# johndpope/OmniHuman-1-hack

Measured on AMD Instinct MI355X. Metric: DiT denoising steps/sec + VAE frames/sec, Wan2.1-1.3B 480x832 81f, higher is better.
Workload: dtype bf16; 1 GPU; Wan2.1-T2V-1.3B 50-step sample, 81f 480x832, latent [16, 21, 60, 104], S=32760, CFG step; weights=random-init (xavier) Wan2.1-T2V-1.3B architecture, parallelism=dp1: replicas, one clip per GPU, no data-path collective

## Files before the change

### omnihuman-1-hack_amd/csrc/dit_elementwise.hip

```cpp
#include "omh_common.h"
#include <mutex>
#include <stdio.h>
#include <string.h>
#include <stdlib.h>

namespace {

constexpr int MAXV_GENERIC = 32;

template <int MAXV, int LN_RPW>
__global__ __launch_bounds__(256)
void layernorm_modulate_kernel(const float* __restrict__ x, uint16_t* __restrict__ y, int64_t rows, int dim,
                               float eps, float mul_const, const float* __restrict__ mul0,
                               const float* __restrict__ mul1, int64_t mul1_stride,
                               const float* __restrict__ add0, const float* __restrict__ add1,
                               int64_t add1_stride, int64_t rows_per_batch) {
    const int lane = threadIdx.x & 63;
    const int64_t row0 = ((int64_t)blockIdx.x * 4 + (threadIdx.x >> 6)) * LN_RPW;
    if (row0 >= rows) return;
    const int nv = dim >> 2;
    float4 mu[MAXV], ad[MAXV], v[MAXV], nx[MAXV];
    int64_t have = -1;
#pragma unroll
    for (int i = 0; i < MAXV; ++i) {
// ... 111 lines not shown
    const float4* wv = (const float4*)weight;
    uint2* yr = (uint2*)(y + row * dim);
    const bool same_pairs = rot && (256 % head_dim) == 0;
    float cs2[2] = {1.f, 1.f}, sn2[2] = {0.f, 0.f};
    if (same_pairs) {
        const int p0 = ((4 * lane) % head_dim) >> 1;
#pragma unroll
        for (int e = 0; e < 2; ++e) {
            const int pc = p0 + e;
            const int pos = pc < cf ? pf : (pc < cf + c3 ? ph : pw);
            const int idx = min(pos, rope_len - 1) * hc + pc;
            cs2[e] = rope_cos[idx]; sn2[e] = rope_sin[idx];
        }
    }
#pragma unroll
    for (int i = 0; i < MAXV; ++i) {
        const int c = lane + 64 * i;
        if (c < nv) {
            float4 t = v[i];
            t.x *= rinv; t.y *= rinv; t.z *= rinv; t.w *= rinv;
            if (wv) { const float4 g = wv[c]; t.x *= g.x; t.y *= g.y; t.z *= g.z; t.w *= g.w; }
            if (rot) {
                const int p0 = ((4 * c) % head_dim) >> 1;
#pragma unroll
                for (int e = 0; e < 2; ++e) {
                    const int pc = p0 + e;
                    const int pos = pc < cf ? pf : (pc < cf + c3 ? ph : pw);
                    const int idx = min(pos, rope_len - 1) * hc + pc;
                    const float cs = same_pairs ? cs2[e] : rope_cos[idx], sn = same_pairs ? sn2[e] : rope_sin[idx];
                    float& re = e == 0 ? t.x : t.z;
                    float& im = e == 0 ? t.y : t.w;
                    const float nr = re * cs - im * sn;
                    const float ni = re * sn + im * cs;
                    re = nr; im = ni;
                }
            }
            uint2 o;
            o.x = pack_bf2(t.x, t.y);
            o.y = pack_bf2(t.z, t.w);
            yr[c] = o;
        }
    }
}

template <int MAXV, bool IN_BF16>
__global__ __launch_bounds__(256)
void rmsnorm_rope_kernel(const void* __restrict__ xv, int64_t ldx, uint16_t* __restrict__ y, int64_t rows,
                         int dim, const float* __restrict__ weight, float eps, int do_norm,
                         const float* __restrict__ rope_cos, const float* __restrict__ rope_sin,
                         int rope_len, int head_dim, const int* __restrict__ grid, int seq_len, float out_scale) {
    rmsnorm_rope_row<MAXV, IN_BF16>(xv, ldx, y, rows, dim, weight, eps, do_norm, rope_cos, rope_sin, rope_len, head_dim, grid,
                                    seq_len, out_scale);
}

template <int MAXV>
__global__ __launch_bounds__(256)
void rmsnorm_rope_pair_kernel(const uint16_t* __restrict__ x, int64_t ldx, int64_t seg_x, uint16_t* __restrict__ y0,
                              uint16_t* __restrict__ y1, int64_t rows, int dim, const float* __restrict__ w0,
                              const float* __restrict__ w1, float eps, int do_norm, const float* __restrict__ rope_cos,
                              const float* __restrict__ rope_sin, int rope_len, int head_dim,
                              const int* __restrict__ grid, int seq_len, float scale0, float scale1) {
    const bool s = blockIdx.y != 0;
    rmsnorm_rope_row<MAXV, true>(x + (s ? seg_x : 0), ldx, s ? y1 : y0, rows, dim, s ? w1 : w0, eps, do_norm, rope_cos, rope_sin,
                                 rope_len, head_dim, grid, seq_len, s ? scale1 : scale0);
}

template <int MAXV>
__global__ __launch_bounds__(256)
void rmsnorm_rope_pair_row_kernel(const uint16_t* __restrict__ x, int64_t ldx, int64_t seg_x, uint16_t* __restrict__ y0,
                                  uint16_t* __restrict__ y1, int64_t rows, int dim, const float* __restrict__ w0,
                                  const float* __restrict__ w1, float eps, int do_norm, const float* __restrict__ rope_cos,
                                  const float* __restrict__ rope_sin, int rope_len, int head_dim,
                                  const int* __restrict__ grid, int seq_len, float scale0, float scale1) {
    const int lane = threadIdx.x & 63;
    const int64_t row = (int64_t)blockIdx.x * 4 + (threadIdx.x >> 6);
    if (row >= rows) return;
    const int nv = dim >> 2;
    const uint2* xa = (const uint2*)(x + row * ldx);
    const uint2* xb = (const uint2*)(x + seg_x + row * ldx);
    uint2 ha[MAXV], hb[MAXV];
#pragma unroll
    for (int i = 0; i < MAXV; ++i) {
        const int c = lane + 64 * i;
        ha[i] = c < nv ? xa[c] : make_uint2(0u, 0u);
    }
#pragma unroll
    for (int i = 0; i < MAXV; ++i) {
        const int c = lane + 64 * i;
        hb[i] = c < nv ? xb[c] : make_uint2(0u, 0u);
    }
    const int hc = head_dim >> 1, c3 = hc / 3, cf = hc - 2 * c3;
    bool rot = false;
    float cs2[2] = {1.f, 1.f}, sn2[2] = {0.f, 0.f};
    {
        const int b = (int)(row / seq_len), sidx = (int)(row % seq_len);
        const int gf = grid[3 * b], gh = grid[3 * b + 1], gw = grid[3 * b + 2];
        if (sidx < gf * gh * gw) {
            rot = true;
            const int pf = sidx / (gh * gw), ph = (sidx / gw) % gh, pw = sidx % gw;
            const int p0 = ((4 * lane) % head_dim) >> 1;
#pragma unroll
            for (int e = 0; e < 2; ++e) {
                const int pc = p0 + e;
                const int pos = pc < cf ? pf : (pc < cf + c3 ? ph : pw);
                const int idx = min(pos, rope_len - 1) * hc + pc;
                cs2[e] = rope_cos[idx]; sn2[e] = rope_sin[idx];
            }
        }
    }
    auto finish = [&](uint2 (&h)[MAXV], uint16_t* __restrict__ y, const float* __restrict__ weight, float out_scale) {
        float4 v[MAXV];
        float q = 0.f;
#pragma unroll
        for (int i = 0; i < MAXV; ++i) {
            const int c = lane + 64 * i;
            if (c < nv) {
                v[i] = make_float4(bf2f((uint16_t)(h[i].x & 0xffff)), bf2f((uint16_t)(h[i].x >> 16)),
                                   bf2f((uint16_t)(h[i].y & 0xffff)), bf2f((uint16_t)(h[i].y >> 16)));
                q += v[i].x * v[i].x + v[i].y * v[i].y + v[i].z * v[i].z + v[i].w * v[i].w;
            }
        }
        const float rinv = (do_norm ? rsqrtf(wave_sum(q) / dim + eps) : 1.0f) * out_scale;
        const float4* wv = (const float4*)weight;
        uint2* yr = (uint2*)(y + row * dim);
#pragma unroll
        for (int i = 0; i < MAXV; ++i) {
            const int c = lane + 64 * i;
            if (c < nv) {
                float4 t = v[i];
                t.x *= rinv; t.y *= rinv; t.z *= rinv; t.w *= rinv;
                if (wv) { const float4 g = wv[c]; t.x *= g.x; t.y *= g.y; t.z *= g.z; t.w *= g.w; }
                if (rot) {
#pragma unroll
                    for (int e = 0; e < 2; ++e) {
                        const float cs = cs2[e], sn = sn2[e];
                        float& re = e == 0 ? t.x : t.z;
                        float& im = e == 0 ? t.y : t.w;
                        const float nr = re * cs - im * sn;
                        const float ni = re * sn + im * cs;
                        re = nr; im = ni;
                    }
                }
                uint2 o;
                o.x = pack_bf2(t.x, t.y);
                o.y = pack_bf2(t.z, t.w);
                yr[c] = o;
            }
        }
    };
    finish(ha, y0, w0, scale0);
    finish(hb, y1, w1, scale1);
}

template <int MAXV>
__global__ __launch_bounds__(256)
void rmsnorm_rope_pair_row_bound_kernel(const uint16_t* __restrict__ x, int64_t ldx, int64_t seg_x, uint16_t* __restrict__ y0,
                                        uint16_t* __restrict__ y1, int64_t rows, int dim, const float* __restrict__ w0,
                                        const float* __restrict__ w1, float eps, int do_norm,
                                        const float* __restrict__ rope_cos, const float* __restrict__ rope_sin, int rope_len,
                                        int head_dim, const int* __restrict__ grid, int seq_len, float scale0, float scale1,
                                        float* __restrict__ norm2_max) {
    const int lane = threadIdx.x & 63;
    const int64_t row = (int64_t)blockIdx.x * 4 + (threadIdx.x >> 6);
    if (row >= rows) return;
    const int nv = dim >> 2;
    const uint2* xa = (const uint2*)(x + row * ldx);
    const uint2* xb = (const uint2*)(x + seg_x + row * ldx);
    uint2 ha[MAXV], hb[MAXV];
#pragma unroll
    for (int i = 0; i < MAXV; ++i) {
        const int c = lane + 64 * i;
        ha[i] = c < nv ? xa[c] : make_uint2(0u, 0u);
    }
#pragma unroll
    for (int i = 0; i < MAXV; ++i) {
        const int c = lane + 64 * i;
        hb[i] = c < nv ? xb[c] : make_uint2(0u, 0u);
    }
    const int hc = head_dim >> 1, c3 = hc / 3, cf = hc - 2 * c3;
    bool rot = false;
    float cs2[2] = {1.f, 1.f}, sn2[2] = {0.f, 0.f};
    const int b = (int)(row / seq_len);
    {
        const int sidx = (int)(row % seq_len);
        const int gf = grid[3 * b], gh = grid[3 * b + 1], gw = grid[3 * b + 2];
        if (sidx < gf * gh * gw) {
            rot = true;
            const int pf = sidx / (gh * gw), ph = (sidx / gw) % gh, pw = sidx % gw;
            const int p0 = ((4 * lane) % head_dim) >> 1;
#pragma unroll
            for (int e = 0; e < 2; ++e) {
                const int pc = p0 + e;
                const int pos = pc < cf ? pf : (pc < cf + c3 ? ph : pw);
                const int idx = min(pos, rope_len - 1) * hc + pc;
                cs2[e] = rope_cos[idx]; sn2[e] = rope_sin[idx];
            }
        }
    }
    const int heads = dim >> 7;
    auto finish = [&](uint2 (&h)[MAXV], uint16_t* __restrict__ y, const float* __restrict__ weight, float out_scale, int seg) {
        float4 v[MAXV];
        float q = 0.f;
#pragma unroll
        for (int i = 0; i < MAXV; ++i) {
            const int c = lane + 64 * i;
            if (c < nv) {
                v[i] = make_float4(bf2f((uint16_t)(h[i].x & 0xffff)), bf2f((uint16_t)(h[i].x >> 16)),
                                   bf2f((uint16_t)(h[i].y & 0xffff)), bf2f((uint16_t)(h[i].y >> 16)));
                q += v[i].x * v[i].x + v[i].y * v[i].y + v[i].z * v[i].z + v[i].w * v[i].w;
            }
        }
        const float rinv = (do_norm ? rsqrtf(wave_sum(q) / dim + eps) : 1.0f) * out_scale;
        const float4* wv = (const float4*)weight;
        uint2* yr = (uint2*)(y + row * dim);
        constexpr int P = MAXV <= 8 ? 8 : 32;
        float r[P];
#pragma unroll
        for (int i = 0; i < P; ++i) r[i] = 0.f;
#pragma unroll
        for (int i = 0; i < MAXV; ++i) {
            const int c = lane + 64 * i;
            if (c < nv) {
                float4 t = v[i];
                t.x *= rinv; t.y *= rinv; t.z *= rinv; t.w *= rinv;
                if (wv) { const float4 g = wv[c]; t.x *= g.x; t.y *= g.y; t.z *= g.z; t.w *= g.w; }
                if (rot) {
#pragma unroll
                    for (int e = 0; e < 2; ++e) {
                        const float cs = cs2[e], sn = sn2[e];
                        float& re = e == 0 ? t.x : t.z;
                        float& im = e == 0 ? t.y : t.w;
                        const float nr = re * cs - im * sn;
                        const float ni = re * sn + im * cs;
                        re = nr; im = ni;
                    }
                }
                uint2 o;
                o.x = pack_bf2(t.x, t.y);
                o.y = pack_bf2(t.z, t.w);
                yr[c] = o;
                {
                    uint32_t px = o.x, py = o.y;
                    asm volatile("" : "+v"(px), "+v"(py));
                    const float a0 = __uint_as_float(px << 16), a1 = __uint_as_float(px & 0xffff0000u);
                    const float a2 = __uint_as_float(py << 16), a3 = __uint_as_float(py & 0xffff0000u);
                    r[i] = a0 * a0 + a1 * a1 + a2 * a2 + a3 * a3;
                }
            }
        }
        {
            int vi = 0;
            float mine = 0.f;
            if constexpr (P == 32) {
#pragma unroll
                for (int i = 0; i < MAXV; ++i) {
#pragma unroll
                    for (int o = 16; o > 0; o >>= 1) r[i] += __shfl_xor(r[i], o, 64);
                    if ((lane & 31) == i) mine = r[i];
                }
                vi = lane & 31;
            } else {
                int n = P;
#pragma unroll
                for (int o = 16; o > 0; o >>= 1) {
                    if (n > 1) {
                        n >>= 1;
                        const bool up = (lane & o) != 0;
#pragma unroll
                        for (int j = 0; j < n; ++j) {
                            const float keep = up ? r[j + n] : r[j], send = up ? r[j] : r[j + n];
                            r[j] = keep + __shfl_xor(send, o, 64);
                        }
                        vi += up ? n : 0;
                    } else {
                        r[0] += __shfl_xor(r[0], o, 64);
                    }
                }
                mine = r[0];
            }
            const int head = 2 * vi + (lane >> 5);
            if ((lane & (32 / P - 1)) == 0 && vi < MAXV && head < heads) {
                unsigned int* slot = (unsigned int*)norm2_max + ((int64_t)b * heads + head) * 2 + seg;
                const unsigned int bits = __float_as_uint(mine);
                if (bits > __hip_atomic_load(slot, __ATOMIC_RELAXED, __HIP_MEMORY_SCOPE_AGENT)) atomicMax(slot, bits);
            }
        }
    };
    finish(ha, y0, w0, scale0, 0);
    finish(hb, y1, w1, scale1, 1);
}

__global__ __launch_bounds__(256)
void cast_f32_bf16_kernel(const float* __restrict__ x, uint16_t* __restrict__ y, int64_t n) {
    const int64_t nv = n >> 2;
    const int64_t stride = (int64_t)gridDim.x * blockDim.x;
    for (int64_t i = (int64_t)blockIdx.x * blockDim.x + threadIdx.x; i < nv; i += stride) {
        const float4 t = ((const float4*)x)[i];
        uint2 o;
        o.x = pack_bf2(t.x, t.y);
        o.y = pack_bf2(t.z, t.w);
        ((uint2*)y)[i] = o;
    }
    if (blockIdx.x == 0 && threadIdx.x < (n & 3)) {
        const int64_t i = (nv << 2) + threadIdx.x;
        y[i] = f2bf(x[i]);
    }
}

__global__ __launch_bounds__(256)
void patchify_kernel(const float* __restrict__ x, uint16_t* __restrict__ tok, int C, int F, int H, int W,
                     int pt, int ph, int pw, int Kp) {
    const int gf = F / pt, gh = H / ph, gw = W / pw;
    const int64_t total = (int64_t)gf * gh * gw * Kp;
    const int kvalid = C * pt * ph * pw;
    const int64_t stride = (int64_t)gridDim.x * blockDim.x;
    for (int64_t i = (int64_t)blockIdx.x * blockDim.x + threadIdx.x; i < total; i += stride) {
        const int k = (int)(i % Kp);
        const int64_t s = i / Kp;
        float val = 0.f;
        if (k < kvalid) {
            const int j = k % pw, ii = (k / pw) % ph, a = (k / (pw * ph)) % pt, c = k / (pw * ph * pt);
            const int w = (int)(s % gw), h = (int)((s / gw) % gh), f = (int)(s / ((int64_t)gw * gh));
            val = x[(((int64_t)c * F + f * pt + a) * H + h * ph + ii) * W + w * pw + j];
        }
        tok[i] = f2bf(val);
    }
}

__global__ __launch_bounds__(256)
void unpatchify_kernel(const float* __restrict__ tok, float* __restrict__ out, int Cout, int gf, int gh, int gw,
                       int pt, int ph, int pw) {
    const int F = gf * pt, H = gh * ph, W = gw * pw;
    const int64_t total = (int64_t)Cout * F * H * W;
    const int ncol = pt * ph * pw * Cout;
    const int64_t stride = (int64_t)gridDim.x * blockDim.x;
    for (int64_t i = (int64_t)blockIdx.x * blockDim.x + threadIdx.x; i < total; i += stride) {
        const int ww = (int)(i % W), hh = (int)((i / W) % H), ff = (int)((i / ((int64_t)W * H)) % F);
        const int c = (int)(i / ((int64_t)W * H * F));
        const int w = ww / pw, j = ww % pw, h = hh / ph, ii = hh % ph, f = ff / pt, a = ff % pt;
        const int64_t s = ((int64_t)f * gh + h) * gw + w;
        out[i] = tok[s * ncol + ((a * ph + ii) * pw + j) * Cout + c];
    }
}

__global__ __launch_bounds__(256)
void dense_f32_kernel(const float* __restrict__ x, const float* __restrict__ W, const float* __restrict__ bias,
                      float* __restrict__ y, int B, int N, int K, int act_in, int act_out) {
    const int lane = threadIdx.x & 63;
    const int64_t o = (int64_t)blockIdx.x * 4 + (threadIdx.x >> 6);
    if (o >= (int64_t)B * N) return;
    const int b = (int)(o / N), n = (int)(o % N);
    const float* xr = x + (int64_t)b * K;
    const float* wr = W + (int64_t)n * K;
    float s = 0.f;
    for (int k = lane; k < K; k += 64) {
        float xv = xr[k];
        if (act_in == 1) xv = xv / (1.0f + expf(-xv));
        s = fmaf(xv, wr[k], s);
    }
    s = wave_sum(s);
    if (lane == 0) {
        if (bias) s += bias[n];
        if (act_out == 1) s = s / (1.0f + expf(-s));
        y[o] = s;
    }
}

__global__ void sinusoid_kernel(const float* __restrict__ t, float* __restrict__ out, int B, int dim) {
    const int half = dim / 2;
    const int i = blockIdx.x * blockDim.x + threadIdx.x;
    if (i >= B * half) return;
    const int b = i / half, k = i % half;
    const double ang = (double)t[b] * pow(10000.0, -(double)k / (double)half);
    out[(int64_t)b * dim + k] = (float)cos(ang);
    out[(int64_t)b * dim + half + k] = (float)sin(ang);
}

__global__ __launch_bounds__(256)
void cfg_unipc_kernel(const float* __restrict__ cond, const float* __restrict__ uncond, const float* x,
                      const float* last, const float* __restrict__ m1, const float* __restrict__ m2,
                      float* __restrict__ mt_out, float* xc_out, float* x_next, int64_t n, float guide, float sigma,
                      int use_corr, float ca_last, float ca_m1, float ca_m2, float ca_mt, float pb_x, float pb_mt,
                      float pb_m1) {
    const int64_t stride = (int64_t)gridDim.x * blockDim.x;
    for (int64_t i = (int64_t)blockIdx.x * blockDim.x + threadIdx.x; i < n; i += stride) {
        const float u = uncond[i];
        const float v = u + guide * (cond[i] - u);
        const float xv = x[i];
        const float mt = xv - sigma * v;
        const float a1 = m1 ? m1[i] : 0.f;
        float xc = xv;
        if (use_corr) {
            xc = ca_last * last[i] + ca_mt * mt;
            if (m1) xc += ca_m1 * a1;
            if (m2) xc += ca_m2 * m2[i];
        }
        float xn = pb_x * xc + pb_mt * mt;
        if (m1) xn += pb_m1 * a1;
        if (mt_out) mt_out[i] = mt;
        if (xc_out) xc_out[i] = xc;
        x_next[i] = xn;
    }
}

template <bool BWD>
__device__ __forceinline__ void flow_x0_one(float v, float x, float e, float s, float s2, bool nxt, float& x0, float& xn) {
    if (BWD) { x0 = -s * v; xn = 0.f; return; }
    float sv = s * v;
    asm volatile("" : "+v"(sv));
    x0 = x - sv;
    float a = (1.f - s2) * x0, b = s2 * e;
    asm volatile("" : "+v"(a), "+v"(b));
    xn = nxt ? a + b : 0.f;
}
template <bool BWD>
__global__ __launch_bounds__(256)
void flow_x0_step_kernel(const float* v, const float* x, const float* eps, const float* __restrict__ sigma,
                         const float* __restrict__ sigma_next, float* x0, float* x_next, int64_t n, int64_t total,
                         int vec_ok) {
    const int64_t stride = (int64_t)gridDim.x * blockDim.x;
    const int64_t tid = (int64_t)blockIdx.x * blockDim.x + threadIdx.x;
    const bool nxt = !BWD && x_next != nullptr;
    const int64_t nvec = vec_ok ? total / 4 : 0;
    for (int64_t i = tid; i < nvec; i += stride) {
        const int64_t e0 = 4 * i;
        const float4 vv = *(const float4*)(v + e0);
        const float4 xv = BWD ? make_float4(0.f, 0.f, 0.f, 0.f) : *(const float4*)(x + e0);
        const float4 ev = nxt ? *(const float4*)(eps + e0) : make_float4(0.f, 0.f, 0.f, 0.f);
        const float va[4] = {vv.x, vv.y, vv.z, vv.w}, xa[4] = {xv.x, xv.y, xv.z, xv.w}, ea[4] = {ev.x, ev.y, ev.z, ev.w};
        float o0[4], o1[4];
        int64_t b = e0 / n, r = e0 - b * n;
#pragma unroll
        for (int k = 0; k < 4; ++k) {
            while (r >= n) { r -= n; ++b; }
            flow_x0_one<BWD>(va[k], xa[k], ea[k], sigma[b], nxt ? sigma_next[b] : 0.f, nxt, o0[k], o1[k]);
            ++r;
        }
        *(float4*)(x0 + e0) = make_float4(o0[0], o0[1], o0[2], o0[3]);
        if (nxt) *(float4*)(x_next + e0) = make_float4(o1[0], o1[1], o1[2], o1[3]);
    }
    for (int64_t i = 4 * nvec + tid; i < total; i += stride) {
        const int64_t b = i / n;
        float a0, a1;
        flow_x0_one<BWD>(v[i], BWD ? 0.f : x[i], nxt ? eps[i] : 0.f, sigma[b], nxt ? sigma_next[b] : 0.f, nxt, a0, a1);
        x0[i] = a0;
        if (nxt) x_next[i] = a1;
    }
}

inline int grid_for(int64_t n, int per_block) {
    int64_t g = (n + per_block - 1) / per_block;
    return (int)(g < 1 ? 1 : (g > 8192 ? 8192 : g));
}

}

extern "C" int omh_layernorm_modulate(const float* x, void* y, int64_t rows, int32_t dim, float eps,
                                      float mul_const, const float* mul0, const float* mul1, int64_t mul1_stride,
                                      const float* add0, const float* add1, int64_t add1_stride,
                                      int64_t rows_per_batch, omh_stream_t stream) {
    if (!x || !y || rows <= 0 || dim <= 0 || rows_per_batch <= 0) return OMH_E_BADARG;
    if ((dim & 3) || dim > MAXV_GENERIC * 256) return OMH_E_SHAPE;
    if (((uintptr_t)x & 15) || ((uintptr_t)y & 7) || (mul1_stride & 3) || (add1_stride & 3)) return OMH_E_ALIGN;
    omh_clear_status();
    const char* force = omh_opt(OMH_OPT_LN_RPW);
    int rpw = rows <= 4096 ? 1 : (rows < 16384 ? 2 : (rows < 24576 ? 4 : 16));
    if (force) { const int f = atoi(force); rpw = (f == 1 || f == 2 || f == 8 || f == 16) ? f : 4; }
#define OMH_LN_PICK(MV) (rpw == 1 ? layernorm_modulate_kernel<MV, 1> : (rpw == 2 ? layernorm_modulate_kernel<MV, 2> : \
                         (rpw == 8 ? layernorm_modulate_kernel<MV, 8> : (rpw == 16 ? layernorm_modulate_kernel<MV, 16> : layernorm_modulate_kernel<MV, 4>))))
    auto kern = dim <= 6 * 256 ? OMH_LN_PICK(6) : (dim <= 20 * 256 ? OMH_LN_PICK(20) : OMH_LN_PICK(MAXV_GENERIC));
#undef OMH_LN_PICK
    hipLaunchKernelGGL(kern, dim3((unsigned)((rows + 4 * rpw - 1) / (4 * rpw))), dim3(256), 0,
                       (hipStream_t)stream, x, (uint16_t*)y, rows, dim, eps, mul_const, mul0, mul1, mul1_stride,
                       add0, add1, add1_stride, rows_per_batch);
    return omh_launch_status();
}

template <bool IN_BF16>
static int rmsnorm_rope_launch(const void* x, int64_t ldx, void* y, int64_t rows, int32_t dim, const float* weight,
                               float eps, int32_t do_norm, const float* rope_cos, const float* rope_sin,
                               int32_t rope_len, int32_t head_dim, const int32_t* grid, int32_t seq_len,
                               float out_scale, omh_stream_t stream) {
    if (!x || !y || rows <= 0 || dim <= 0) return OMH_E_BADARG;
    if ((dim & 3) || dim > MAXV_GENERIC * 256 || (ldx & 3)) return OMH_E_SHAPE;
    if (rope_cos && (!rope_sin || !grid || seq_len <= 0 || head_dim <= 0 || (head_dim & 3) || dim % head_dim))
        return OMH_E_BADARG;
    if (((uintptr_t)x & (IN_BF16 ? 7 : 15)) || ((uintptr_t)y & 7)) return OMH_E_ALIGN;
    omh_clear_status();
    auto kern = dim <= 6 * 256 ? rmsnorm_rope_kernel<6, IN_BF16>
                               : (dim <= 20 * 256 ? rmsnorm_rope_kernel<20, IN_BF16> : rmsnorm_rope_kernel<MAXV_GENERIC, IN_BF16>);
    hipLaunchKernelGGL(kern, dim3((unsigned)((rows + 3) / 4)), dim3(256), 0, (hipStream_t)stream,
                       x, ldx, (uint16_t*)y, rows, dim, weight, eps, do_norm, rope_cos, rope_sin, rope_len,
                       head_dim, grid, seq_len, out_scale);
    return omh_launch_status();
}

extern "C" int omh_rmsnorm_rope(const float* x, int64_t ldx, void* y, int64_t rows, int32_t dim,
                                const float* weight, float eps, int32_t do_norm, const float* rope_cos,
                                const float* rope_sin, int32_t rope_len, int32_t head_dim, const int32_t* grid,
                                int32_t seq_len, omh_stream_t stream) {
    return rmsnorm_rope_launch<false>(x, ldx, y, rows, dim, weight, eps, do_norm, rope_cos, rope_sin, rope_len,
                                      head_dim, grid, seq_len, 1.0f, stream);
}

extern "C" int omh_rmsnorm_rope_bf16(const void* x_bf16, int64_t ldx, void* y, int64_t rows, int32_t dim,
                                     const float* weight, float eps, int32_t do_norm, const float* rope_cos,
                                     const float* rope_sin, int32_t rope_len, int32_t head_dim,
                                     const int32_t* grid, int32_t seq_len, float out_scale, omh_stream_t stream) {
    return rmsnorm_rope_launch<true>(x_bf16, ldx, y, rows, dim, weight, eps, do_norm, rope_cos, rope_sin, rope_len,
                                     head_dim, grid, seq_len, out_scale, stream);
}

extern "C" int omh_rmsnorm_rope_bf16_pair(const void* x_bf16, int64_t ldx, int64_t seg_x, void* y0, void* y1, int64_t rows,
                                          int32_t dim, const float* weight0, const float* weight1, float eps, int32_t do_norm,
                                          const float* rope_cos, const float* rope_sin, int32_t rope_len, int32_t head_dim,
                                          const int32_t* grid, int32_t seq_len, float out_scale0, float out_scale1,
                                          omh_stream_t stream) {
    if (!x_bf16 || !y0 || !y1 || rows <= 0 || dim <= 0) return OMH_E_BADARG;
    if ((dim & 3) || dim > MAXV_GENERIC * 256 || (ldx & 3) || (seg_x & 3)) return OMH_E_SHAPE;
    if (rope_cos && (!rope_sin || !grid || seq_len <= 0 || head_dim <= 0 || (head_dim & 3) || dim % head_dim))
        return OMH_E_BADARG;
    if (((uintptr_t)x_bf16 & 7) || ((uintptr_t)y0 & 7) || ((uintptr_t)y1 & 7)) return OMH_E_ALIGN;
    omh_clear_status();
    {
        const char* pr = omh_opt(OMH_OPT_RMS_PAIR_ROW);
        const bool off = pr && pr[0] == '0', on = pr && pr[0] == '1';
        if (!off && rope_cos && head_dim > 0 && (256 % head_dim) == 0 && dim <= 20 * 256 && (on || rows >= 8192)) {
            auto k2 = dim <= 6 * 256 ? rmsnorm_rope_pair_row_kernel<6> : rmsnorm_rope_pair_row_kernel<20>;
            hipLaunchKernelGGL(k2, dim3((unsigned)((rows + 3) / 4)), dim3(256), 0, (hipStream_t)stream,
                               (const uint16_t*)x_bf16, ldx, seg_x, (uint16_t*)y0, (uint16_t*)y1, rows, dim, weight0, weight1,
                               eps, do_norm, rope_cos, rope_sin, rope_len, head_dim, grid, seq_len, out_scale0, out_scale1);
            return omh_launch_status();
        }
    }
    auto kern = dim <= 6 * 256 ? rmsnorm_rope_pair_kernel<6>
                               : (dim <= 20 * 256 ? rmsnorm_rope_pair_kernel<20> : rmsnorm_rope_pair_kernel<MAXV_GENERIC>);
    hipLaunchKernelGGL(kern, dim3((unsigned)((rows + 3) / 4), 2), dim3(256), 0, (hipStream_t)stream,
                       (const uint16_t*)x_bf16, ldx, seg_x, (uint16_t*)y0, (uint16_t*)y1, rows, dim, weight0, weight1, eps,
                       do_norm, rope_cos, rope_sin, rope_len, head_dim, grid, seq_len, out_scale0, out_scale1);
    return omh_launch_status();
}

extern "C" int omh_rmsnorm_rope_bf16_pair_bound(const void* x_bf16, int64_t ldx, int64_t seg_x, void* y0, void* y1,
                                                int64_t rows, int32_t dim, const float* weight0, const float* weight1,
                                                float eps, int32_t do_norm, const float* rope_cos, const float* rope_sin,
                                                int32_t rope_len, int32_t head_dim, const int32_t* grid, int32_t seq_len,
                                                float out_scale0, float out_scale1, float* norm2_max, omh_stream_t stream) {
    if (!x_bf16 || !y0 || !y1 || !norm2_max || rows <= 0 || dim <= 0) return OMH_E_BADARG;
    if (!rope_cos || !rope_sin || !grid || seq_len <= 0) return OMH_E_BADARG;
    if ((dim & 3) || (ldx & 3) || (seg_x & 3) || head_dim != 128 || dim % 128 || dim > 20 * 256) return OMH_E_SHAPE;
    if (((uintptr_t)x_bf16 & 7) || ((uintptr_t)y0 & 7) || ((uintptr_t)y1 & 7) || ((uintptr_t)norm2_max & 3)) return OMH_E_ALIGN;
    omh_clear_status();
    auto k2 = dim <= 6 * 256 ? rmsnorm_rope_pair_row_bound_kernel<6> : rmsnorm_rope_pair_row_bound_kernel<20>;
    hipLaunchKernelGGL(k2, dim3((unsigned)((rows + 3) / 4)), dim3(256), 0, (hipStream_t)stream, (const uint16_t*)x_bf16, ldx,
                       seg_x, (uint16_t*)y0, (uint16_t*)y1, rows, dim, weight0, weight1, eps, do_norm, rope_cos, rope_sin,
                       rope_len, head_dim, grid, seq_len, out_scale0, out_scale1, norm2_max);
    return omh_launch_status();
}

extern "C" int omh_cast_f32_bf16(const float* x, void* y, int64_t n, omh_stream_t stream) {
    if (!x || !y || n <= 0) return OMH_E_BADARG;
    if (((uintptr_t)x & 15) || ((uintptr_t)y & 7)) return OMH_E_ALIGN;
    omh_clear_status();
    hipLaunchKernelGGL(cast_f32_bf16_kernel, dim3(grid_for(n / 4 + 1, 256)), dim3(256), 0, (hipStream_t)stream,
                       x, (uint16_t*)y, n);
    return omh_launch_status();
}

extern "C" int omh_patchify(const float* x, void* tok, int32_t C, int32_t F, int32_t H, int32_t W, int32_t pt,
                            int32_t ph, int32_t pw, int32_t Kp, omh_stream_t stream) {
    if (!x || !tok || C <= 0 || F <= 0 || H <= 0 || W <= 0 || pt <= 0 || ph <= 0 || pw <= 0) return OMH_E_BADARG;
    if (F % pt || H % ph || W % pw || Kp < C * pt * ph * pw) return OMH_E_SHAPE;
    const int64_t total = (int64_t)(F / pt) * (H / ph) * (W / pw) * Kp;
    omh_clear_status();
    hipLaunchKernelGGL(patchify_kernel, dim3(grid_for(total, 256)), dim3(256), 0, (hipStream_t)stream, x,
                       (uint16_t*)tok, C, F, H, W, pt, ph, pw, Kp);
    return omh_launch_status();
}

extern "C" int omh_unpatchify(const float* tok, float* out, int32_t Cout, int32_t f, int32_t h, int32_t w,
                              int32_t pt, int32_t ph, int32_t pw, omh_stream_t stream) {
    if (!tok || !out || Cout <= 0 || f <= 0 || h <= 0 || w <= 0 || pt <= 0 || ph <= 0 || pw <= 0)
        return OMH_E_BADARG;
    const int64_t total = (int64_t)Cout * f * pt * h * ph * w * pw;
    omh_clear_status();
    hipLaunchKernelGGL(unpatchify_kernel, dim3(grid_for(total, 256)), dim3(256), 0, (hipStream_t)stream, tok, out,
                       Cout, f, h, w, pt, ph, pw);
    return omh_launch_status();
}

extern "C" int omh_dense_f32(const float* x, const float* W, const float* bias, float* y, int32_t B, int32_t N,
                             int32_t K, int32_t act_in, int32_t act_out, omh_stream_t stream) {
    if (!x || !W || !y || B <= 0 || N <= 0 || K <= 0) return OMH_E_BADARG;
    const int64_t outs = (int64_t)B * N;
    omh_clear_status();
    hipLaunchKernelGGL(dense_f32_kernel, dim3((unsigned)((outs + 3) / 4)), dim3(256), 0, (hipStream_t)stream, x, W,
                       bias, y, B, N, K, act_in, act_out);
    return omh_launch_status();
}

extern "C" int omh_sinusoidal_embedding(const float* t, float* out, int32_t B, int32_t dim, omh_stream_t stream) {
    if (!t || !out || B <= 0 || dim <= 0 || (dim & 1)) return OMH_E_BADARG;
    const int n = B * (dim / 2);
    omh_clear_status();
    hipLaunchKernelGGL(sinusoid_kernel, dim3((n + 255) / 256), dim3(256), 0, (hipStream_t)stream, t, out, B, dim);
    return omh_launch_status();
}

extern "C" int omh_cfg_unipc_step(const float* cond, const float* uncond, const float* x, const float* last,
                                  const float* m1, const float* m2, float* mt_out, float* xc_out, float* x_next,
                                  int64_t n, float guide, float sigma, int32_t use_corr, float ca_last, float ca_m1,
                                  float ca_m2, float ca_mt, float pb_x, float pb_mt, float pb_m1,
                                  omh_stream_t stream) {
    if (!cond || !uncond || !x || !x_next || n <= 0) return OMH_E_BADARG;
    if (use_corr && !last) return OMH_E_BADARG;
    omh_clear_status();
    hipLaunchKernelGGL(cfg_unipc_kernel, dim3(grid_for(n, 256)), dim3(256), 0, (hipStream_t)stream, cond, uncond, x,
                       last, m1, m2, mt_out, xc_out, x_next, n, guide, sigma, use_corr, ca_last, ca_m1, ca_m2, ca_mt,
                       pb_x, pb_mt, pb_m1);
    return omh_launch_status();
}

extern "C" int omh_flow_x0_step(const float* v, const float* x, const float* eps, const float* sigma, const float* sigma_next,
                                float* x0, float* x_next, int32_t B, int64_t n, int32_t backward, omh_stream_t stream) {
    if (!v || !sigma || !x0 || B <= 0 || n <= 0) return OMH_E_BADARG;
    if (!backward && !x) return OMH_E_BADARG;
    if (!backward && x_next && (!eps || !sigma_next)) return OMH_E_BADARG;
    const int64_t total = (int64_t)B * n;
    if (((uintptr_t)v | (uintptr_t)x | (uintptr_t)eps | (uintptr_t)x0 | (uintptr_t)x_next) & 3) return OMH_E_ALIGN;
    uintptr_t al = (uintptr_t)v | (uintptr_t)x0;
    if (!backward) al |= (uintptr_t)x | (x_next ? ((uintptr_t)x_next | (uintptr_t)eps) : 0);
    const int vec_ok = (al & 15) == 0;
    omh_clear_status();
    const int grid = grid_for((total + 3) / 4, 256);
    if (backward)
        hipLaunchKernelGGL(flow_x0_step_kernel<true>, dim3(grid), dim3(256), 0, (hipStream_t)stream, v, x, eps, sigma,
                           sigma_next, x0, x_next, n, total, vec_ok);
    else
        hipLaunchKernelGGL(flow_x0_step_kernel<false>, dim3(grid), dim3(256), 0, (hipStream_t)stream, v, x, eps, sigma,
                           sigma_next, x0, x_next, n, total, vec_ok);
    return omh_launch_status();
}

namespace {
const char* const g_opt_name[OMH_OPT_COUNT] = {
#define X(n) #n,
    OMH_OPTIONS(X)
#undef X
};
char g_opt_val[OMH_OPT_COUNT][48];
char g_opt_env[OMH_OPT_COUNT][48];
int g_deterministic = 0, g_deterministic_env = 0;
std::once_flag g_opt_once;

void opt_store(char* dst, const char* v) {
    size_t n = v ? strlen(v) : 0;
    if (n > 47) n = 47;
    if (n) memcpy(dst, v, n);
    dst[n] = 0;
}
void opt_init() {
    std::call_once(g_opt_once, [] {
        char name[64];
        for (int i = 0; i < OMH_OPT_COUNT; ++i) {
            snprintf(name, sizeof name, "OMH_%s", g_opt_name[i]);
            opt_store(g_opt_env[i], getenv(name));
            opt_store(g_opt_val[i], g_opt_env[i]);
        }
        const char* e = getenv("OMH_DETERMINISTIC");
        g_deterministic = g_deterministic_env = (e && e[0] == '1') ? 1 : 0;
    });
}
int opt_index(const char* key) {
    if (!key) return -1;
    if (!strncmp(key, "OMH_", 4)) key += 4;
    for (int i = 0; i < OMH_OPT_COUNT; ++i)
        if (!strcmp(key, g_opt_name[i])) return i;
    return -1;
}
}

const char* omh_opt(int id) {
    opt_init();
    return g_opt_val[id][0] ? g_opt_val[id] : nullptr;
}
extern "C" int omh_set_option(const char* key, const char* value) {
    opt_init();
    if (!key) {
        if (value) return OMH_E_BADARG;
        for (int i = 0; i < OMH_OPT_COUNT; ++i) opt_store(g_opt_val[i], g_opt_env[i]);
        g_deterministic = g_deterministic_env;
        return 0;
    }
    if (!strcmp(key, "DETERMINISTIC") || !strcmp(key, "OMH_DETERMINISTIC")) {
        g_deterministic = (value && value[0] == '1') ? 1 : 0;
        return 0;
    }
    const int i = opt_index(key);
    if (i < 0) return OMH_E_BADARG;
    if (value && strlen(value) > 47) return OMH_E_SHAPE;
    opt_store(g_opt_val[i], value);
    return 0;
}
extern "C" const char* omh_get_option(const char* key) {
    opt_init();
// ... 20 lines not shown
```

### omnihuman-1-hack_amd/csrc/omh_common.h

```cpp
#pragma once
#include <hip/hip_runtime.h>
#include <stdint.h>
#include <type_traits>

#include "../../include/omh.h"

#define OMH_OPTIONS(X)                                                                                                   \
    X(ATTN_KERNEL) X(ATTN_SPLIT) X(W64_SPLIT) X(W64_VARIANT) X(CONV_PERSIST) X(CONV_W64_UP2) X(LN_RPW) X(GEMM_GROUP_M)    \
    X(GEMM_TILE) X(GEMM_RULE) X(GEMM_KERNEL) X(GEMM_W64_GBWD) X(GEMM_W64_GAUX) X(GEMM_W64_R192) X(GEMM_W64_BF16M)        \
    X(GEMM_W64_N192) X(GEMM_TN_SPLIT) X(GEMM_TN_W64) X(GEMM_TN_TILE) X(GEMM_TN_GROUP_TILE) X(GEMM_SPLITK) X(CONV_TILE)   \
    X(CONV_WIDE_MIN) X(CONV_W64) X(CONV_FUSE_NORM) X(CONV_KW3) X(GEMM_QKV) X(ATTN_BWD_W64) X(GEMM_W64_P256) X(RMS_PAIR_ROW)  \
    X(ATTN_BOUNDED)
enum OmhOpt {
#define X(n) OMH_OPT_##n,
    OMH_OPTIONS(X)
#undef X
    OMH_OPT_COUNT
};
const char* omh_opt(int id);

typedef __attribute__((ext_vector_type(8))) __bf16 bf16x8;
typedef __attribute__((ext_vector_type(4))) __bf16 bf16x4;
typedef __attribute__((ext_vector_type(16))) float f32x16;
typedef __attribute__((ext_vector_type(4))) float f32x4;
typedef __attribute__((ext_vector_type(4))) uint32_t u32x4;

#define OMH_WAVE 64

__device__ __forceinline__ uint16_t f2bf(float f) {
    uint32_t u = __float_as_uint(f);
    if ((u & 0x7fffffffu) > 0x7f800000u) return (uint16_t)((u >> 16) | 0x40u);
    u += 0x7fffu + ((u >> 16) & 1u);
    return (uint16_t)(u >> 16);
}
__device__ __forceinline__ float bf2f(uint16_t h) { return __uint_as_float(((uint32_t)h) << 16); }

typedef float omh_f32x2 __attribute__((ext_vector_type(2)));
typedef __bf16 omh_bf16x2 __attribute__((ext_vector_type(2)));
__device__ __forceinline__ uint32_t pack_bf2(float lo, float hi) {
    const omh_f32x2 v = {lo, hi};
    return __builtin_bit_cast(uint32_t, __builtin_convertvector(v, omh_bf16x2));
}
__device__ __forceinline__ float fast_exp2(float x) { return __builtin_amdgcn_exp2f(x); }

__device__ __forceinline__ float gelu_tanh(float x) {
    const float x2 = x * x;
    const float k = -2.0f * 0.7978845608028654f * 1.4426950408889634f;
    const float t = k * x * fmaf(0.044715f, x2, 1.0f);
    return x * __builtin_amdgcn_rcpf(1.0f + __builtin_amdgcn_exp2f(t));
}
__device__ __forceinline__ float gelu_tanh_grad(float x) {
    const float c = 0.7978845608028654f, a = 0.044715f;
    const float x2 = x * x;
    const float k = -2.0f * c * 1.4426950408889634f;
    const float s = __builtin_amdgcn_rcpf(1.0f + __builtin_amdgcn_exp2f(k * x * fmaf(a, x2, 1.0f)));
    return fmaf(x * (2.0f * c) * fmaf(3.0f * a, x2, 1.0f), s * (1.0f - s), s);
}
__device__ __forceinline__ float silu(float x) {
    return x * __builtin_amdgcn_rcpf(1.0f + __builtin_amdgcn_exp2f(-1.4426950408889634f * x));
}

__device__ __forceinline__ float wave_sum(float v) {
#pragma unroll
    for (int o = 32; o > 0; o >>= 1) v += __shfl_xor(v, o, 64);
    return v;
}

__device__ __forceinline__ int xcd_remap(int bid, int nwg) {
    const int nx = 8;
    const int q = nwg / nx, r = nwg % nx;
    const int xcd = bid % nx, idx = bid / nx;
    const int base = (xcd < r) ? xcd * (q + 1) : r * (q + 1) + (xcd - r) * q;
    return base + idx;
}

__device__ __forceinline__ void tile_of(int wid, int tiles_m, int tiles_n, int& tm, int& tn, const int GM = 8) {
    const int per_group = GM * tiles_n;
    const int gid = wid / per_group, in_g = wid - gid * per_group;
    const int first_m = gid * GM;
    const int gsz = min(tiles_m - first_m, GM);
    tm = first_m + in_g % gsz;
    tn = in_g / gsz;
}

__global__ __launch_bounds__(256) static void omh_zero_f32_kernel(float* __restrict__ p, int64_t rows, int64_t cols,
                                                                  int64_t ld) {
    const int64_t n = rows * cols;
    for (int64_t i = (int64_t)blockIdx.x * blockDim.x + threadIdx.x; i < n; i += (int64_t)gridDim.x * blockDim.x)
        p[(i / cols) * ld + (i % cols)] = 0.f;
}
static inline void omh_zero_f32(float* p, int64_t rows, int64_t cols, int64_t ld, hipStream_t s) {
    const int64_t n = rows * cols;
    int64_t g = (n + 255) / 256;
    g = g < 1 ? 1 : (g > 4096 ? 4096 : g);
    hipLaunchKernelGGL(omh_zero_f32_kernel, dim3((unsigned)g), dim3(256), 0, s, p, rows, cols, ld);
}

bool omh_deterministic();

static inline void omh_clear_status() { (void)hipGetLastError(); }
static inline int omh_launch_status() {
    hipError_t e = hipGetLastError();
    return e == hipSuccess ? 0 : (int)e;
}


struct BlkList {
    const int32_t* cnt;
    const int32_t* idx;
    int heads, lists, stride;
};
static inline int omh_block_mask_check(const omh_block_mask* m, int H, int Lq, int Lk) {
    if (!m->row_cnt || !m->row_idx || !m->col_cnt || !m->col_idx) return OMH_E_BADARG;
    if (m->heads != 1 && m->heads != H) return OMH_E_BADARG;
    if (m->q_blocks != (Lq + 127) / 128 || m->k_blocks != (Lk + 127) / 128) return OMH_E_BADARG;
    if (((uintptr_t)m->row_cnt | (uintptr_t)m->row_idx | (uintptr_t)m->col_cnt | (uintptr_t)m->col_idx) & 3) return OMH_E_ALIGN;
    return 0;
}
static inline bool omh_mask_window_unset(int wl, int wr) { return (wl < 0 && wr < 0) || (wl == 0 && wr == 0); }

struct ChunkRule {
    int chunk, left, off;
};
static inline int omh_chunk_rule(const omh_chunk_causal* c, int Lq, int Lk, ChunkRule* out) {
    if (!c || c->chunk <= 0 || c->q_offset < 0 || c->reserved != 0) return OMH_E_BADARG;
    const int64_t span = (int64_t)c->q_offset + Lq;
    if (span + Lk >= (1LL << 28)) return OMH_E_SHAPE;
    const int64_t cap = span > Lk ? span : Lk;
    out->chunk = c->chunk > cap ? (int)cap : c->chunk;
    const int64_t reach = span / out->chunk + 1;
    out->left = c->left_chunks < 0 ? -1 : (c->left_chunks > reach ? (int)reach : c->left_chunks);
    out->off = c->q_offset;
    return 0;
}

struct IvlTab {
    const int32_t* iv;
    int group, n, other;
};
static inline BlkList omh_ivl_arg(const int32_t* iv, int group, int n, int other) { return BlkList{nullptr, iv, group, n, other}; }
static_assert(sizeof(BlkList) == 2 * sizeof(void*) + 4 * sizeof(int) && sizeof(IvlTab) + sizeof(void*) == sizeof(BlkList),
              "IvlTab travels in a BlkList: one pointer and three ints beside the unused cnt");
static_assert(std::is_same<decltype(BlkList::idx), decltype(IvlTab::iv)>::value && std::is_same<decltype(BlkList::heads), int>::value &&
              std::is_same<decltype(BlkList::lists), int>::value && std::is_same<decltype(BlkList::stride), int>::value,
              "omh_ivl_arg / omh_ivl_tab map idx, heads, lists, stride to iv, group, n, other");
static inline int omh_interval_mask_check(const omh_interval_mask* m, int Lq, int Lk) {
    if (!m || !m->q_iv || !m->k_iv || m->group < 8 || m->reserved != 0) return OMH_E_BADARG;
    if ((int64_t)Lq + Lk >= (1LL << 28)) return OMH_E_SHAPE;
    if (m->q_groups != (Lq + m->group - 1) / m->group || m->k_groups != (Lk + m->group - 1) / m->group) return OMH_E_BADARG;
    if (((uintptr_t)m->q_iv | (uintptr_t)m->k_iv) & 3) return OMH_E_ALIGN;
    return 0;
}
static inline int omh_interval3_mask_check(const omh_interval3_mask* m, int Lq, int Lk) {
    if (!m || !m->q_iv || !m->k_iv || m->group < 8 || m->reserved != 0) return OMH_E_BADARG;
    if ((int64_t)Lq + Lk >= (1LL << 28)) return OMH_E_SHAPE;
    if (m->q_groups != (Lq + m->group - 1) / m->group || m->k_groups != (Lk + m->group - 1) / m->group) return OMH_E_BADARG;
    if (((uintptr_t)m->q_iv | (uintptr_t)m->k_iv) & 3) return OMH_E_ALIGN;
    return 0;
}
#if defined(__HIPCC__)
__device__ __forceinline__ IvlTab omh_ivl_tab(const BlkList& bl) { return IvlTab{bl.idx, bl.heads, bl.lists, bl.stride}; }
struct IvlSpan {
    int lo0, len0, lo1, len1;
    __device__ __forceinline__ bool sees(int x) const {
        return (unsigned)(x - lo0) < (unsigned)len0 || (unsigned)(x - lo1) < (unsigned)len1;
// ... 124 lines not shown
```

Before: 2.350 denoising steps/s (1 step = 2 DiT forwards, CFG).

## Add persistent double-buffered RMSNorm+RoPE pair kernel with per-batch norm-max folding

Adds a persistent, grid-strided variant of the bounded q/k RMSNorm+RoPE kernel for dim=1536. Each wave prefetches the next row into registers while it finishes the current one. The kernel stages the gains in LDS with the pair order swapped, uses packed f32 math, and keeps a running per-head norm maximum so the atomicMax is issued only when the batch changes. This targets launch and tail overhead, load latency, and contention on the per-row atomics. In exchange it adds inline asm complexity and fixes occupancy at waves_per_eu 4. It also adds compile-time ablation hooks to the old kernel and env options to select the old form or cap the workgroup count.

New measurement: 2.369 denoising steps/s (1 step = 2 DiT forwards, CFG) (median of 6 runs). No clear change (+0.8%).

```diff
diff --git a/omnihuman-1-hack_amd/csrc/dit_elementwise.hip b/omnihuman-1-hack_amd/csrc/dit_elementwise.hip
--- a/omnihuman-1-hack_amd/csrc/dit_elementwise.hip
+++ b/omnihuman-1-hack_amd/csrc/dit_elementwise.hip
@@ -287,6 +287,9 @@
     finish(hb, y1, w1, scale1);
 }
 
+#ifndef OMH_RMS_ABL
+#define OMH_RMS_ABL 0
+#endif
 template <int MAXV>
 __global__ __launch_bounds__(256)
 void rmsnorm_rope_pair_row_bound_kernel(const uint16_t* __restrict__ x, int64_t ldx, int64_t seg_x, uint16_t* __restrict__ y0,
@@ -333,6 +336,16 @@
         }
     }
     const int heads = dim >> 7;
+#if OMH_RMS_ABL == 2
+    unsigned int early[2];
+    {
+        const int vi = ((lane >> 4) & 1) * 4 + ((lane >> 3) & 1) * 2 + ((lane >> 2) & 1);
+        const int head = min(2 * vi + (lane >> 5), heads - 1);
+        unsigned int* slot = (unsigned int*)norm2_max + ((int64_t)b * heads + head) * 2;
+        early[0] = __hip_atomic_load(slot, __ATOMIC_RELAXED, __HIP_MEMORY_SCOPE_AGENT);
+        early[1] = __hip_atomic_load(slot + 1, __ATOMIC_RELAXED, __HIP_MEMORY_SCOPE_AGENT);
+    }
+#endif
     auto finish = [&](uint2 (&h)[MAXV], uint16_t* __restrict__ y, const float* __restrict__ weight, float out_scale, int seg) {
         float4 v[MAXV];
         float q = 0.f;
@@ -417,12 +430,205 @@
             if ((lane & (32 / P - 1)) == 0 && vi < MAXV && head < heads) {
                 unsigned int* slot = (unsigned int*)norm2_max + ((int64_t)b * heads + head) * 2 + seg;
                 const unsigned int bits = __float_as_uint(mine);
+#if OMH_RMS_ABL == 1
+                (void)slot;
+                asm volatile("" : : "v"(bits));
+#elif OMH_RMS_ABL == 2
+                if (bits > early[seg]) atomicMax(slot, bits);
+#else
                 if (bits > __hip_atomic_load(slot, __ATOMIC_RELAXED, __HIP_MEMORY_SCOPE_AGENT)) atomicMax(slot, bits);
+#endif
             }
         }
     };
     finish(ha, y0, w0, scale0, 0);
     finish(hb, y1, w1, scale1, 1);
+}
+
+template <int MAXV>
+__global__ __launch_bounds__(256) __attribute__((amdgpu_waves_per_eu(4)))
+void rmsnorm_rope_pair_stream_bound_kernel(const uint16_t* __restrict__ x, int64_t ldx, int64_t seg_x, uint16_t* __restrict__ y0,
+                                           uint16_t* __restrict__ y1, int64_t rows, int dim, const float* __restrict__ w0,
+                                           const float* __restrict__ w1, float eps, int do_norm,
+                                           const float* __restrict__ rope_cos, const float* __restrict__ rope_sin,
+                                           int rope_len, int head_dim, const int* __restrict__ grid, int seq_len,
+                                           float scale0, float scale1, float* __restrict__ norm2_max) {
+    static_assert(MAXV <= 8, "the half-wave exchange below is the 8-value one");
+    const int lane = threadIdx.x & 63;
+    const int heads = MAXV * 2;
+    __shared__ float4 gains[2][MAXV * 64];
+    for (int c = threadIdx.x; c < MAXV * 64; c += 256) {
+        const float4 t0 = w0 ? ((const float4*)w0)[c] : make_float4(1.f, 1.f, 1.f, 1.f);
+        const float4 t1 = w1 ? ((const float4*)w1)[c] : make_float4(1.f, 1.f, 1.f, 1.f);
+        gains[0][c] = make_float4(t0.x, t0.z, t0.y, t0.w);
+        gains[1][c] = make_float4(t1.x, t1.z, t1.y, t1.w);
+    }
+    __syncthreads();
+    const int W = (int)gridDim.x * 4;
+    const int w = __builtin_amdgcn_readfirstlane((int)blockIdx.x * 4 + (int)(threadIdx.x >> 6));
+    if (w >= rows) return;
+    const int hc = head_dim >> 1, c3 = hc / 3, cf = hc - 2 * c3;
+    const int p0 = ((4 * lane) % head_dim) >> 1;
+    const int vi = ((lane >> 4) & 1) * 4 + ((lane >> 3) & 1) * 2 + ((lane >> 2) & 1);
+    const int head = 2 * vi + (lane >> 5);
+    const bool holder = (lane & 3) == 0 && vi < MAXV && head < heads;
+    int have = -1, gf = 0, gh = 1, gw = 1;
+    auto fetch = [&](int64_t row, int b, int sidx, uint2 (&a)[MAXV], uint2 (&bb)[MAXV], float (&cs)[2], float (&sn)[2],
+                     bool& rot) __attribute__((always_inline)) {
+        const uint2* xa = (const uint2*)(x + row * ldx);
+        const uint2* xb = (const uint2*)(x + seg_x + row * ldx);
+#pragma unroll
+        for (int i = 0; i < MAXV; ++i) {
+            const int c = lane + 64 * i;
+            a[i] = xa[c];
+        }
+#pragma unroll
+        for (int i = 0; i < MAXV; ++i) {
+            const int c = lane + 64 * i;
+            bb[i] = xb[c];
+        }
+        if (b != have) { have = b; gf = grid[3 * b]; gh = grid[3 * b + 1]; gw = grid[3 * b + 2]; }
+        rot = sidx < gf * gh * gw;
+        const int ghw = max(gh * gw, 1), gw1 = max(gw, 1);
+        const int pf = sidx / ghw, ph = (sidx / gw1) % max(gh, 1), pw = sidx % gw1;
+#pragma unroll
+        for (int e = 0; e < 2; ++e) {
+            const int pc = p0 + e;
+            const int pos = pc < cf ? pf : (pc < cf + c3 ? ph : pw);
+            const int idx = max(min(pos, rope_len - 1), 0) * hc + pc;
+            cs[e] = rope_cos[idx]; sn[e] = rope_sin[idx];
+        }
+    };
+    auto pk_mul = [](omh_f32x2 x0, omh_f32x2 x1) __attribute__((always_inline)) {
+        omh_f32x2 d;
+        asm("v_pk_mul_f32 %0, %1, %2" : "=v"(d) : "v"(x0), "v"(x1));
+        return d;
+    };
+    auto pk_fma = [](omh_f32x2 x0, omh_f32x2 x1, omh_f32x2 x2) __attribute__((always_inline)) {
+        omh_f32x2 d;
+        asm("v_pk_fma_f32 %0, %1, %2, %3" : "=v"(d) : "v"(x0), "v"(x1), "v"(x2));
+        return d;
+    };
+    auto pk_fms = [](omh_f32x2 x0, omh_f32x2 x1, omh_f32x2 x2) __attribute__((always_inline)) {
+        omh_f32x2 d;
+        asm("v_pk_fma_f32 %0, %1, %2, %3 neg_lo:[0,0,1] neg_hi:[0,0,1]" : "=v"(d) : "v"(x0), "v"(x1), "v"(x2));
+        return d;
+    };
+    auto fma1 = [](float x0, float x1, float x2) __attribute__((always_inline)) {
+        float d;
+        asm("v_fma_f32 %0, %1, %2, %3" : "=v"(d) : "v"(x0), "v"(x1), "v"(x2));
+        return d;
+    };
+    auto finish = [&](uint2 (&h)[MAXV], uint16_t* __restrict__ y, const float4* g, float out_scale, int64_t row,
+                      bool rot, const float (&cs2)[2], const float (&sn2)[2]) __attribute__((always_inline)) -> unsigned int {
+        float q = 0.f;
+#pragma unroll
+        for (int i = 0; i < MAXV; ++i) {
+            const omh_f32x2 P = {__uint_as_float(h[i].x << 16), __uint_as_float(h[i].y << 16)};
+            const omh_f32x2 Q = {__uint_as_float(h[i].x & 0xffff0000u), __uint_as_float(h[i].y & 0xffff0000u)};
+            const omh_f32x2 P2 = pk_mul(P, P), Q2 = pk_mul(Q, Q);
+            q = q + (((P2.x + Q2.x) + P2.y) + Q2.y);
+        }
+        const float rinv = (do_norm ? rsqrtf(wave_sum(q) / dim + eps) : 1.0f) * out_scale;
+        const omh_f32x2 rr = {rinv, rinv}, cs = {cs2[0], cs2[1]}, sn = {sn2[0], sn2[1]};
+        uint2* yr = (uint2*)(y + row * dim);
+        float r[8];
+#pragma unroll
+        for (int i = 0; i < 8; ++i) r[i] = 0.f;
+#pragma unroll
+        for (int i = 0; i < MAXV; ++i) {
+            const int c = lane + 64 * i;
+            asm volatile("" : "+v"(h[i].x), "+v"(h[i].y));
+            omh_f32x2 P = {__uint_as_float(h[i].x << 16), __uint_as_float(h[i].y << 16)};
+            omh_f32x2 Q = {__uint_as_float(h[i].x & 0xffff0000u), __uint_as_float(h[i].y & 0xffff0000u)};
+            const float4 gi = g[c];
+            const omh_f32x2 gp = {gi.x, gi.y}, gq = {gi.z, gi.w};
+            P = pk_mul(pk_mul(P, rr), gp);
+            Q = pk_mul(pk_mul(Q, rr), gq);
+            if (rot) {
+                const omh_f32x2 nr = pk_fms(P, cs, pk_mul(Q, sn)), ni = pk_fma(Q, cs, pk_mul(P, sn));
+                P = nr; Q = ni;
+            }
+            uint2 o;
+            o.x = pack_bf2(P.x, Q.x);
+            o.y = pack_bf2(P.y, Q.y);
+            yr[c] = o;
+            {
+                uint32_t px = o.x, py = o.y;
+                asm volatile("" : "+v"(px), "+v"(py));
+                const omh_f32x2 A = {__uint_as_float(px << 16), __uint_as_float(py << 16)};
+                const omh_f32x2 Bv = {__uint_as_float(px & 0xffff0000u), __uint_as_float(py & 0xffff0000u)};
+                const omh_f32x2 A2 = pk_mul(A, A), B2 = pk_mul(Bv, Bv);
+                if (i == 2 || i == 4)
+                    r[i] = fma1(Bv.y, Bv.y, A2.y + fma1(A.x, A.x, B2.x));
+                else
+                    r[i] = ((A2.x + B2.x) + A2.y) + B2.y;
+            }
+            __builtin_amdgcn_sched_barrier(0);
+        }
+        int n = 8;
+#pragma unroll
+        for (int o = 16; o > 0; o >>= 1) {
+            if (n > 1) {
+                n >>= 1;
+                const bool up = (lane & o) != 0;
+#pragma unroll
+                for (int j = 0; j < n; ++j) {
+                    float lo = r[j], hi = r[j + n];
+                    asm("" : "+v"(lo), "+v"(hi));
+                    const float keep = up ? hi : lo, send = up ? lo : hi;
+                    r[j] = keep + __shfl_xor(send, o, 64);
+                }
+            } else {
+                r[0] += __shfl_xor(r[0], o, 64);
+            }
+        }
+        return __float_as_uint(r[0]);
+    };
+
+    uint2 qa[MAXV], ka[MAXV], qb[MAXV], kb[MAXV];
+    float cs_a[2], sn_a[2], cs_b[2], sn_b[2];
+    bool rot_a, rot_b = false;
+    int64_t row = w;
+    int b = w / seq_len, sidx = w % seq_len;
+    fetch(row, b, sidx, qa, ka, cs_a, sn_a, rot_a);
+    unsigned int run0 = 0u, run1 = 0u;
+    auto step = [&](uint2 (&hq)[MAXV], uint2 (&hk)[MAXV], const float (&cs)[2], const float (&sn)[2], bool rot,
+                    uint2 (&nq)[MAXV], uint2 (&nk)[MAXV], float (&ncs)[2], float (&nsn)[2],
+                    bool& nrot) __attribute__((always_inline)) -> bool {
+        asm volatile("" ::: "memory");
+        const int64_t nrow = row + W;
+        const bool more = nrow < rows;
+        int bn = b, sidx_n = sidx + W;
+        if (more) {
+            if (sidx_n >= seq_len) { const int adv = sidx_n / seq_len; bn += adv; sidx_n -= adv * seq_len; }
+            fetch(nrow, bn, sidx_n, nq, nk, ncs, nsn, nrot);
+        }
+        const bool flush = !more || bn != b, fold = flush && holder;
+        unsigned int* slot = (unsigned int*)norm2_max + ((int64_t)b * heads + (holder ? head : 0)) * 2;
+        unsigned int cur0, cur1;
+        if (fold) {
+            cur0 = __hip_atomic_load(slot, __ATOMIC_RELAXED, __HIP_MEMORY_SCOPE_AGENT);
+            cur1 = __hip_atomic_load(slot + 1, __ATOMIC_RELAXED, __HIP_MEMORY_SCOPE_AGENT);
+        }
+        __builtin_amdgcn_sched_barrier(0);
+        run0 = max(run0, finish(hq, y0, gains[0], scale0, row, rot, cs, sn));
+        __builtin_amdgcn_sched_barrier(0);
+        run1 = max(run1, finish(hk, y1, gains[1], scale1, row, rot, cs, sn));
+        __builtin_amdgcn_sched_barrier(0);
+        if (fold) {
+            if (run0 > cur0) atomicMax(slot, run0);
+            if (run1 > cur1) atomicMax(slot + 1, run1);
+        }
+        if (flush) run0 = run1 = 0u;
+        row = nrow; b = bn; sidx = sidx_n;
+        return more;
+    };
+    if (!step(qa, ka, cs_a, sn_a, rot_a, qb, kb, cs_b, sn_b, rot_b)) return;
+    for (;;) {
+        if (!step(qb, kb, cs_b, sn_b, rot_b, qa, ka, cs_a, sn_a, rot_a)) break;
+        if (!step(qa, ka, cs_a, sn_a, rot_a, qb, kb, cs_b, sn_b, rot_b)) break;
+    }
 }
 
 __global__ __launch_bounds__(256)
@@ -686,6 +892,18 @@
     if ((dim & 3) || (ldx & 3) || (seg_x & 3) || head_dim != 128 || dim % 128 || dim > 20 * 256) return OMH_E_SHAPE;
     if (((uintptr_t)x_bf16 & 7) || ((uintptr_t)y0 & 7) || ((uintptr_t)y1 & 7) || ((uintptr_t)norm2_max & 3)) return OMH_E_ALIGN;
     omh_clear_status();
+    const char* form = omh_opt(OMH_OPT_RMS_BOUND_FORM);
+    if (dim == 6 * 256 && !(form && !strcmp(form, "row"))) {
+        int64_t wgs = (rows + 3) / 4;
+        const int64_t full = (int64_t)omh_cu_count() * 4;
+        if (wgs > full) wgs = full;
+        const char* cap = omh_opt(OMH_OPT_RMS_BOUND_WGS);
+        if (cap && atoi(cap) > 0 && wgs > atoi(cap)) wgs = atoi(cap);
+        hipLaunchKernelGGL(rmsnorm_rope_pair_stream_bound_kernel<6>, dim3((unsigned)wgs), dim3(256), 0, (hipStream_t)stream,
+                           (const uint16_t*)x_bf16, ldx, seg_x, (uint16_t*)y0, (uint16_t*)y1, rows, dim, weight0, weight1, eps,
+                           do_norm, rope_cos, rope_sin, rope_len, head_dim, grid, seq_len, out_scale0, out_scale1, norm2_max);
+        return omh_launch_status();
+    }
     auto k2 = dim <= 6 * 256 ? rmsnorm_rope_pair_row_bound_kernel<6> : rmsnorm_rope_pair_row_bound_kernel<20>;
     hipLaunchKernelGGL(k2, dim3((unsigned)((rows + 3) / 4)), dim3(256), 0, (hipStream_t)stream, (const uint16_t*)x_bf16, ldx,
                        seg_x, (uint16_t*)y0, (uint16_t*)y1, rows, dim, weight0, weight1, eps, do_norm, rope_cos, rope_sin,
diff --git a/omnihuman-1-hack_amd/csrc/omh_common.h b/omnihuman-1-hack_amd/csrc/omh_common.h
--- a/omnihuman-1-hack_amd/csrc/omh_common.h
+++ b/omnihuman-1-hack_amd/csrc/omh_common.h
@@ -10,7 +10,7 @@
     X(GEMM_TILE) X(GEMM_RULE) X(GEMM_KERNEL) X(GEMM_W64_GBWD) X(GEMM_W64_GAUX) X(GEMM_W64_R192) X(GEMM_W64_BF16M)        \
     X(GEMM_W64_N192) X(GEMM_TN_SPLIT) X(GEMM_TN_W64) X(GEMM_TN_TILE) X(GEMM_TN_GROUP_TILE) X(GEMM_SPLITK) X(CONV_TILE)   \
     X(CONV_WIDE_MIN) X(CONV_W64) X(CONV_FUSE_NORM) X(CONV_KW3) X(GEMM_QKV) X(ATTN_BWD_W64) X(GEMM_W64_P256) X(RMS_PAIR_ROW)  \
-    X(ATTN_BOUNDED)
+    X(ATTN_BOUNDED) X(RMS_BOUND_FORM) X(RMS_BOUND_WGS)
 enum OmhOpt {
 #define X(n) OMH_OPT_##n,
     OMH_OPTIONS(X)
```
